# joeyee/Onet

Hardware: AMD Instinct MI355X
Metric: training images/sec (twin 256x256 pass) (higher is better)
Workload: dtype f32

## Files before the change

### include/onet_hip.h

```cpp
#ifndef ONET_HIP_H
#define ONET_HIP_H

#include <stdint.h>

#ifdef __cplusplus
extern "C" {
#endif

#define ONET_OK 0
#define ONET_EINVAL (-1)
#define ONET_EHIP (-2)

const char* onet_last_error(void);
int onet_abi_version(void);
int onet_device_info(int* cu_count, int* lds_bytes, int* wave_size, char* arch, int arch_len);

int onet_conv3x3_pack_weights(const float* w, float* wp_fwd, float* wp_dgrad,
                              int Cout, int Cin, void* stream);
int onet_convT2x2_pack_weights(const float* w, float* wp_fwd, float* wp_dgrad,
                               int Cin, int Cout, void* stream);
int onet_convT2x2_pack_weights_fused(const float* w, float* wq, int Cin, int Cout, void* stream);
int onet_convT2x2_fwd(const float* x, int64_t x_bs, const float* wq, const float* bias, float* y, int64_t y_bs,
                      int B, int Cin, int Ct, int h, int w, int Ho, int Wo, int pt, int pl, int operand_bf16,
        void* stream);
// ... 116 lines not shown
int onet_bn_bwd_finalize(const float* part2, int nparts, int64_t count, float* dgamma, float* dbeta, float* coef, int accumulate,
                         int groups, int C, const float* save, const void* da_amax, void* dz_amax, void* stream);
int onet_bn_bwd_finalize_cm(const float* part2, int nparts, int64_t c_stride, int64_t count, float* dgamma,
                            float* dbeta, float* coef, int accumulate, int C, void* stream);
int onet_bn_relu_bwd_apply(const float* da, int64_t da_bs, const float* z, int64_t z_bs, const float* save, const float* coef,
                           float* dz, int64_t dz_bs, void* amax, int group_images, int B, int C, int HW, void* stream);
int onet_bn_relu_apply_split(const void* z, int z_bf16, int64_t z_bs, void* xs, int64_t xs_bs, float* a, int64_t a_bs, const float* save,
                             const void* act_amax, int nparts, int group_images, int B, int C, int H, int W, void* stream);
int onet_bn_relu_apply_pool_split(const void* z, int z_bf16, int64_t z_bs, void* xs, int64_t xs_bs, float* a, int64_t a_bs, void* ys, int64_t ys_bs,
                                  float* y, int64_t y_bs, const float* save, const void* act_amax, int nparts, int group_images, int B, int C,
                                  int H, int W, void* stream);
int onet_bn_bwd_bound(const float* save, const float* coef, const void* da_amax, int64_t count, void* dz_amax, int C, void* stream);
int onet_bn_relu_bwd_apply_split(const float* da, int64_t da_bs, const void* z, int z_bf16, int64_t z_bs, const float* save, const float* coef,
                                 void* dzs, int64_t dzs_bs, const void* dz_amax, int nparts, int group_images, int B, int C, int H, int W,
                                 void* stream);

int onet_maxpool2_fwd(const float* x, int64_t x_bs, float* y, int64_t y_bs,
                      int B, int C, int H, int W, void* stream);
int onet_maxpool2_bwd(const float* x, int64_t x_bs, const float* dy, int64_t dy_bs, const float* add, int64_t add_bs,
                      const float* add2, int64_t add2_bs, float* dx, int64_t dx_bs, int B, int C, int H, int W, int accumulate,
                      void* stream);
int onet_maxpool2_bwd_bn_bands(int H, int W);
int onet_maxpool2_bwd_add_bnreduce(const float* x, int64_t x_bs, const float* dy, int64_t dy_bs, const float* add, int64_t add_bs,
                                        const float* add2, int64_t add2_bs, float* dx, int64_t dx_bs, const void* z, int z_bf16, int64_t z_bs,
                                        const float* save, int group_images, float* part2, void* dx_amax, int B, int C, int H, int W,
                                        void* stream);

int onet_pixel_shuffle2_bias(const float* sub, const float* bias, float* y, int64_t y_bs,
                             int B, int C, int h, int w, int Ho, int Wo, int pt, int pl, void* stream);
int onet_space_to_depth2(const float* dy, int64_t dy_bs, float* sub, float* dbias, double* scratch,
// ... 5 lines not shown
int onet_bilinear2x_fwd(const float* x, int64_t x_bs, float* y, int64_t y_bs, int B, int C,
                        int h, int w, int Ho, int Wo, int pt, int pl, void* stream);
int onet_bilinear2x_bwd(const float* dy, int64_t dy_bs, float* dx, int64_t dx_bs, int B, int C,
                        int h, int w, int Ho, int Wo, int pt, int pl, void* stream);

int onet_complement_clip(const float* x, float* y, float bias, int64_t n, void* stream);

int onet_head_softmax_fwd(const float* Lt, int64_t Lt_bs, const float* Ht, int64_t Ht_bs, const float* Ld, int64_t Ld_bs, const float* Hd,
                          int64_t Hd_bs, float* Vt, float* Vd, float* S, float* sLt, float* sLd, const float* h_save_t, const float* h_save_d,
                          int B, int C, int HW, void* stream);
int onet_head_softmax_bwd(const float* dVt, const float* dVd, const float* dS, const float* gsLt, const float* gsLd, const float* S,
                          const float* Lt, int64_t Lt_bs, const float* Ht, int64_t Ht_bs, const float* Ld, int64_t Ld_bs, const float* Hd,
                          int64_t Hd_bs, float* dLt, float* dHt, float* dLd, float* dHd, const float* h_save_t, const float* h_save_d, int B,
                          int C, int HW, void* stream);

int onet_jsd_fwd(const float* L, int64_t L_bs, const float* Si, int64_t Si_bs,
                 const float* Sp, int64_t Sp_bs, float* sums, double* part, float* jsd,
                 int B, int C, int HW, void* stream);
int onet_jsd_nparts(void);
int onet_jsd_bwd(const float* gscale, const float* sums, const float* Si, int64_t Si_bs,
                 const float* Sp, int64_t Sp_bs, float* gL, float* dSi, float* dSp,
                 int B, int HW, void* stream);
int onet_log1pexp_inplace(float* x, int64_t n, void* stream);
int onet_log1pexp_bwd(const float* x, const float* g, float* out, int64_t n, void* stream);

int onet_argmax2(const float* S, int64_t* Y, int B, int HW, void* stream);

int onet_normalise_per_frame(const float* x, float* y, int planes, int HW, void* stream);

int onet_clutter_fft_size(void);
// ... 21 lines not shown
```

### onet_amd/csrc/bn.hip

```cpp
#include <type_traits>
#include "common.hpp"

using namespace onet;

__global__ __launch_bounds__(256) void bn_stats_partial_kernel(const float* __restrict__ z, int64_t z_bs,
                                                               float* __restrict__ part, int C, int HW,
                                                               int chunks, int chunk_len) {
    __shared__ double red[16];
    const int c = blockIdx.x % C;
    const int p = blockIdx.x / C;
    const int b = p / chunks, ch = p % chunks;
    const float* src = z + (int64_t)b * z_bs + (int64_t)c * HW;
    const int beg = ch * chunk_len;
    const int end = min(beg + chunk_len, HW);
    const bool vec = ((HW & 3) == 0) && ((z_bs & 3) == 0) && ((chunk_len & 3) == 0);
    const double pivot = (double)src[beg];
    double v[2] = {0.0, 0.0};
    if (vec) {
        int i = beg + threadIdx.x * 4;
        for (; i + 3072 < end; i += 4096) {
            float4 q[4];
#pragma unroll
            for (int k = 0; k < 4; ++k) q[k] = *reinterpret_cast<const float4*>(src + i + 1024 * k);
#pragma unroll
// ... 459 lines not shown
    }
    if (!live) return;
    if (ys) {
        unsigned* o = ys + (int64_t)b * ys_bs;
        bn_store_slots(o, ((int64_t)(c8 * Hp + yo) * np) * Wp + 2 * q, Wp, m[0], s_act, np);
        bn_store_slots(o, ((int64_t)(c8 * Hp + yo) * np) * Wp + 2 * q + 1, Wp, m[1], s_act, np);
    }
    if (yf) {
        float* d = yf + (int64_t)b * yf_bs + (int64_t)c8 * 8 * Hp * Wp + (int64_t)yo * Wp + 2 * q;
#pragma unroll
        for (int k = 0; k < 8; ++k) *reinterpret_cast<float2*>(d + (int64_t)k * Hp * Wp) = make_float2(m[0][k], m[1][k]);
    }
}

constexpr int BN_BWD_OCC16 = 4;
template <typename ZT = float>
__global__ __launch_bounds__(256, sizeof(ZT) == 2 ? BN_BWD_OCC16 : 3) void bn_relu_bwd_apply_split_kernel(const float* __restrict__ da, int64_t da_bs, const ZT* __restrict__ z,
                                                                      int64_t z_bs, const float* __restrict__ save, const float* __restrict__ coef,
                                                                      unsigned* __restrict__ dzs, int64_t dzs_bs, const unsigned* __restrict__ slots,
                                                                      int C, int H, int W, int bpp, int np, int gimg) {
    float inv;
    const float s = np == 1 ? 1.f : amax_scale(amax_read(slots), true, inv);
    const int plane = blockIdx.x / bpp, blk = blockIdx.x % bpp;
    const int C8 = C >> 3, b = plane / C8, c8 = plane % C8;
    if (gimg) {
        save += (int64_t)(b / gimg) * 4 * C;
        if (coef) coef += (int64_t)(b / gimg) * 4 * C;
    }
    bn_u32x4* const tr = bn_tr_lds();
    const int HW = H * W, p = (blk * 256 + threadIdx.x) * 4;
    const bool live = p < HW;
    const ZT* zs = z + (int64_t)b * z_bs + (int64_t)c8 * 8 * HW + p;
    const float* ds = da + (int64_t)b * da_bs + (int64_t)c8 * 8 * HW + p;
    constexpr bool Z16 = sizeof(ZT) == 2;
    typename std::conditional<Z16, uint2, float4>::type zq[8];
    float4 gq[8];
#pragma unroll
    for (int k = 0; k < 8; ++k) {
        if constexpr (Z16) zq[k] = live ? *reinterpret_cast<const uint2*>(zs + (int64_t)k * HW) : make_uint2(0u, 0u);
        else zq[k] = live ? *reinterpret_cast<const float4*>(zs + (int64_t)k * HW) : make_float4(0.f, 0.f, 0.f, 0.f);
        gq[k] = live ? *reinterpret_cast<const float4*>(ds + (int64_t)k * HW) : make_float4(0.f, 0.f, 0.f, 0.f);
    }
    float v[4][8];
#pragma unroll
    for (int k = 0; k < 8; ++k) {
        const int c = c8 * 8 + k;
        const float mean = save[c], invstd = save[C + c], sc = save[2 * C + c], sh = save[3 * C + c];
        const double c1 = coef ? (double)coef[c] + (double)coef[C + c] : 0.0;
        const double c2 = coef ? (double)coef[2 * C + c] + (double)coef[3 * C + c] : 0.0;
        float zz[4];
        if constexpr (Z16) {
            zz[0] = __builtin_bit_cast(float, zq[k].x << 16); zz[1] = __builtin_bit_cast(float, zq[k].x & 0xffff0000u);
            zz[2] = __builtin_bit_cast(float, zq[k].y << 16); zz[3] = __builtin_bit_cast(float, zq[k].y & 0xffff0000u);
        } else {
            zz[0] = zq[k].x; zz[1] = zq[k].y; zz[2] = zq[k].z; zz[3] = zq[k].w;
        }
        const float gg[4] = {gq[k].x, gq[k].y, gq[k].z, gq[k].w};
#pragma unroll
        for (int e = 0; e < 4; ++e) {
            const double dy = fmaf(zz[e] - mean, sc, sh) > 0.f ? (double)gg[e] : 0.0;
            v[e][k] = (float)((double)sc * (dy - c1 - (((double)zz[e] - (double)mean) * (double)invstd) * c2));
        }
    }
    bn_store_slots_block(tr, dzs + (int64_t)b * dzs_bs, c8, H, W, blk * 1024, HW, v, s, np);
}

__global__ __launch_bounds__(64) void bn_bwd_bound_kernel(const float* __restrict__ save, const float* __restrict__ coef,
                                                          const unsigned* __restrict__ da_slots, float xhat_max, unsigned* __restrict__ dz_slots,
                                                          int C) {
    const float da_max = amax_read(da_slots);
    float bound = 0.f;
    for (int c = blockIdx.x * 64 + threadIdx.x; c < C; c += gridDim.x * 64) {
// ... 65 lines not shown
            v[1] += dy * (((double)zi - meand) * invd);
            vmax = fmaxf(vmax, fabsf(ds[i]));
        }
    }
    amax_commit(vmax, amax);
    block_sum_256<double, 2>(v, red);
    if (threadIdx.x == 0) {
        float* o = part2 + ((int64_t)p * C + c) * 4;
        o[0] = (float)v[0];
        o[1] = (float)(v[0] - (double)o[0]);
        o[2] = (float)v[1];
        o[3] = (float)(v[1] - (double)o[2]);
    }
}

__global__ __launch_bounds__(256) void bn_bwd_finalize_kernel(const float* __restrict__ part2, int nparts,
                                                             double count, float* dgamma, float* dbeta,
                                                             float* coef, int accumulate, int C, const float* __restrict__ save = nullptr,
                                                             const unsigned* __restrict__ da_slots = nullptr,
                                                             unsigned* __restrict__ dz_slots = nullptr, float xhat_max = 0.f, int groups = 1) {
    __shared__ double wsum[2][4];
    const float da_max = dz_slots ? amax_read(da_slots) : 0.f;
    const int c = blockIdx.x;
    float acc_b = 0.f, acc_g = 0.f;
    if (accumulate && threadIdx.x == 0) {
        acc_b = dbeta ? dbeta[c] : 0.f;
        acc_g = dgamma ? dgamma[c] : 0.f;
    }
    for (int g = 0; g < groups; ++g) {
        const float* rec = part2 + (int64_t)g * nparts * C * 4;
// ... 283 lines not shown
                 "bn_relu_bwd_apply_split: bad args");
    ONET_REQUIRE((reinterpret_cast<uintptr_t>(dzs) & 15) == 0 && (dzs_bs & 3) == 0 && (reinterpret_cast<uintptr_t>(z) & 15) == 0 && (z_bs & 3) == 0 &&
                 (reinterpret_cast<uintptr_t>(da) & 15) == 0 && (da_bs & 3) == 0, "bn_relu_bwd_apply_split: 16-byte aligned rows and slots required");
    const int bpp = cdiv((int64_t)H * W, 1024);
    const int64_t blocks = (int64_t)B * (C / 8) * bpp;
    ONET_REQUIRE(blocks < (1ll << 31) && (int64_t)H * W < (1 << 24), "bn_relu_bwd_apply_split: grid too large");
    if (z_bf16)
        hipLaunchKernelGGL(bn_relu_bwd_apply_split_kernel<__bf16>, dim3((unsigned)blocks), dim3(256), bn_tr_bytes(nparts), as_stream(stream), da, da_bs,
                           (const __bf16*)z, z_bs, save, coef, (unsigned*)dzs, dzs_bs, (const unsigned*)dz_amax, C, H, W, bpp, nparts, group_images);
    else
        hipLaunchKernelGGL(bn_relu_bwd_apply_split_kernel<float>, dim3((unsigned)blocks), dim3(256), bn_tr_bytes(nparts), as_stream(stream), da, da_bs,
                           (const float*)z, z_bs, save, coef, (unsigned*)dzs, dzs_bs, (const unsigned*)dz_amax, C, H, W, bpp, nparts, group_images);
    return check_launch("bn_relu_bwd_apply_split_kernel");
}

int onet_bn_bwd_finalize_cm(const float* part2, int nparts, int64_t c_stride, int64_t count, float* dgamma, float* dbeta,
                            float* coef, int accumulate, int C, void* stream) {
    ONET_REQUIRE(part2 && nparts > 0 && count > 0 && C > 0 && c_stride >= (int64_t)nparts * 2, "bn_bwd_finalize_cm: bad args");
    hipLaunchKernelGGL(bn_bwd_finalize_cm_kernel, dim3(C), dim3(256), 0, as_stream(stream), part2, nparts, c_stride,
                       (double)count, dgamma, dbeta, coef, accumulate, C);
    return check_launch("bn_bwd_finalize_cm_kernel");
}

int onet_bn_bwd_finalize(const float* part2, int nparts, int64_t count, float* dgamma, float* dbeta, float* coef, int accumulate,
                               int groups, int C, const float* save, const void* da_amax, void* dz_amax, void* stream) {
    ONET_REQUIRE(part2 && nparts > 0 && count > 0 && C > 0 && groups >= 1 && (!dz_amax || (save && da_amax)), "bn_bwd_finalize: bad args");
    hipLaunchKernelGGL(bn_bwd_finalize_kernel, dim3(C), dim3(256), 0, as_stream(stream), part2, nparts, (double)count, dgamma, dbeta, coef,
                       accumulate, C, save, (const unsigned*)da_amax, (unsigned*)dz_amax, sqrtf((float)(count > 1 ? count - 1 : 1)), groups);
    return check_launch("bn_bwd_finalize_kernel");
}
// ... 14 lines not shown
```

### onet_amd/csrc/head_loss.hip

```cpp
#include <algorithm>
#include "common.hpp"

using namespace onet;

__device__ __forceinline__ float f_quirk(float x) {
    if (x <= -37.f) return logf(1.f + expf(expf(x)));
    if (x <= 18.f) return logf(1.f + expf(x));
    if (x < 33.3f) return x + expf(-x);
    return x;
}
__device__ __forceinline__ float df_quirk(float x) {
    if (x <= -37.f) {
        const float e = expf(x), ee = expf(e);
        return ee / (1.f + ee) * e;
    }
    if (x <= 18.f) {
        const float e = expf(x);
        return e / (1.f + e);
    }
    if (x < 33.3f) return 1.f - expf(-x);
    return 1.f;
}

__global__ void log1pexp_kernel(float* x, int64_t n) {
// ... 30 lines not shown
            st_ += a;
            sd_ += d;
        }
        Vt[i] = vt;
        Vd[i] = vd;
        if (sLt) sLt[i] = st_;
        if (sLd) sLd[i] = sd_;
        const float m = fmaxf(vt, vd);
        const float et = expf(vt - m), ed = expf(vd - m);
        const float den = et + ed;
        S[((int64_t)b * 2 + 0) * HW + p] = et / den;
        S[((int64_t)b * 2 + 1) * HW + p] = ed / den;
    }
}

__global__ __launch_bounds__(256) void head_softmax_bwd_kernel(
    const float* __restrict__ dVt, const float* __restrict__ dVd, const float* __restrict__ dS,
    const float* __restrict__ S, const float* __restrict__ Lt, int64_t Lt_bs, const float* __restrict__ Ht,
    int64_t Ht_bs, const float* __restrict__ Ld, int64_t Ld_bs, const float* __restrict__ Hd, int64_t Hd_bs,
    float* __restrict__ dLt, float* __restrict__ dHt, float* __restrict__ dLd, float* __restrict__ dHd,
    const float* __restrict__ gsLt, const float* __restrict__ gsLd, const float* __restrict__ nt, const float* __restrict__ nd, int B,
    int C, int HW) {
    const int64_t n = (int64_t)B * HW;
    const int64_t CHW = (int64_t)C * HW;
    for (int64_t i = blockIdx.x * (int64_t)blockDim.x + threadIdx.x; i < n; i += (int64_t)gridDim.x * blockDim.x) {
        const int b = (int)(i / HW);
        const int p = (int)(i % HW);
        float gt = dVt ? dVt[i] : 0.f, gd = dVd ? dVd[i] : 0.f;
        if (dS) {
            const float st = S[((int64_t)b * 2 + 0) * HW + p], sd = S[((int64_t)b * 2 + 1) * HW + p];
            const float a = dS[((int64_t)b * 2 + 0) * HW + p], d = dS[((int64_t)b * 2 + 1) * HW + p];
            const float t = st * sd * (a - d);
            gt += t;
            gd -= t;
        }
        const float* lt = Lt + b * Lt_bs + p;
        const float* ht = Ht + b * Ht_bs + p;
        const float* ld = Ld + b * Ld_bs + p;
        const float* hd = Hd + b * Hd_bs + p;
        float* olt = dLt + b * CHW + p;
        float* oht = dHt + b * CHW + p;
        float* old_ = dLd + b * CHW + p;
        float* ohd = dHd + b * CHW + p;
        const float at = gsLt ? gsLt[i] : 0.f, ad = gsLd ? gsLd[i] : 0.f;
        for (int c = 0; c < C; ++c) {
            const int64_t o = (int64_t)c * HW;
            float h1 = ht[o], h2 = hd[o];
            if (nt) {
                h1 = fmaxf(fmaf(h1 - nt[c], nt[2 * C + c], nt[3 * C + c]), 0.f);
                h2 = fmaxf(fmaf(h2 - nd[c], nd[2 * C + c], nd[3 * C + c]), 0.f);
            }
            olt[o] = fmaf(gt, h1, at);
            oht[o] = gt * lt[o];
            old_[o] = fmaf(gd, h2, ad);
            ohd[o] = gd * ld[o];
        }
    }
}

constexpr int JSD_BLOCKS = 2048;

__global__ __launch_bounds__(256) void jsd_fwd_kernel(const float* __restrict__ L, int64_t L_bs,
                                                      const float* __restrict__ Si, int64_t Si_bs,
                                                      const float* __restrict__ Sp, int64_t Sp_bs,
                                                      float* __restrict__ sums, double* __restrict__ part, int B,
                                                      int C, int HW) {
    __shared__ double red[4];
    const int64_t n = (int64_t)B * HW;
    double acc[1] = {0.0};
    for (int64_t i = blockIdx.x * (int64_t)blockDim.x + threadIdx.x; i < n; i += (int64_t)gridDim.x * blockDim.x) {
        const int b = (int)(i / HW);
        const int p = (int)(i % HW);
        float sl;
        if (L) {
// ... 73 lines not shown
                       Lt_bs, Ht, Ht_bs, Ld, Ld_bs, Hd, Hd_bs, Vt, Vd, S, sLt, sLd, h_save_t, h_save_d, B, C, HW);
    return check_launch("head_softmax_fwd_kernel");
}

int onet_head_softmax_bwd(const float* dVt, const float* dVd, const float* dS, const float* gsLt, const float* gsLd, const float* S,
                          const float* Lt, int64_t Lt_bs, const float* Ht, int64_t Ht_bs, const float* Ld, int64_t Ld_bs, const float* Hd,
                          int64_t Hd_bs, float* dLt, float* dHt, float* dLd, float* dHd, const float* h_save_t, const float* h_save_d, int B,
                          int C, int HW, void* stream) {
    ONET_REQUIRE(S && Lt && Ht && Ld && Hd && dLt && dHt && dLd && dHd && (!h_save_t == !h_save_d) && B > 0 && C > 0 && HW > 0,
                 "head_softmax_bwd: bad args");
    hipLaunchKernelGGL(head_softmax_bwd_kernel, dim3(grid_px((int64_t)B * HW)), dim3(256), 0, as_stream(stream), dVt,
                       dVd, dS, S, Lt, Lt_bs, Ht, Ht_bs, Ld, Ld_bs, Hd, Hd_bs, dLt, dHt, dLd, dHd, gsLt, gsLd, h_save_t, h_save_d, B, C, HW);
    return check_launch("head_softmax_bwd_kernel");
}

int onet_jsd_nparts(void) { return JSD_BLOCKS; }

int onet_jsd_fwd(const float* L, int64_t L_bs, const float* Si, int64_t Si_bs, const float* Sp, int64_t Sp_bs,
                 float* sums, double* part, float* jsd, int B, int C, int HW, void* stream) {
    ONET_REQUIRE(Si && Sp && sums && part && jsd && B > 0 && C > 0 && HW > 0, "jsd_fwd: bad args");
    const int64_t n = (int64_t)B * HW;
    int blocks = (int)std::min<int64_t>((n + 255) / 256, JSD_BLOCKS);
    hipLaunchKernelGGL(jsd_fwd_kernel, dim3(blocks), dim3(256), 0, as_stream(stream), L, L_bs, Si, Si_bs, Sp, Sp_bs,
                       sums, part, B, C, HW);
    int rc = check_launch("jsd_fwd_kernel");
    if (rc) return rc;
    hipLaunchKernelGGL(jsd_final_kernel, dim3(1), dim3(256), 0, as_stream(stream), (const double*)part, blocks,
                       -1.0 / (double)n, jsd);
    return check_launch("jsd_final_kernel");
}
// ... 29 lines not shown
```

### onet_amd/functional.py

```python
from __future__ import annotations

import torch

from . import ops


def _carries_settings(cls):
    fwd, bwd = cls.forward, cls.backward

    def forward(ctx, *args, **kw):
        ctx._onet_settings = ops.active_settings()
        return fwd(ctx, *args, **kw)

    def backward(ctx, *grads):
        if torch.is_grad_enabled():
            raise RuntimeError("onet_amd: double differentiation (create_graph=True) is not supported: the HIP backward kernels "
                               "build no graph of their own")
        with ops.using(getattr(ctx, "_onet_settings", None)):
            return bwd(ctx, *grads)

    forward.__doc__, backward.__doc__ = fwd.__doc__, bwd.__doc__
    cls.forward, cls.backward = staticmethod(forward), staticmethod(backward)
    return cls

# ... 137 lines not shown
            else:
                pooled = (torch.empty((Bz, C, Hz // 2, Wz // 2), dtype=torch.float32, device=z.device), None, None)
        if training and cm is not None:
            ops.bn_train_coeffs(z[:Bg], gamma, beta, running_mean, running_var, momentum, eps, cm=(cm, 0, cm.shape[1] // G), save=save_all,
                                act_slots=act_slots, groups=G)
        else:
            for g in range(G):
                if training:
                    ops.bn_train_coeffs(z[g * Bg:(g + 1) * Bg], gamma, beta, running_mean, running_var, momentum, eps, save=save_all[g],
                                        act_slots=act_slots)
                else:
                    ops.bn_eval_coeffs(gamma, beta, running_mean, running_var, eps, save=save_all[g])
        gi = Bg if G > 1 else 0
        if defer_head:
            head["z"], head["save"] = z, save_all
            a_amax = None
        elif pooled is not None:
            if not ops.bn_relu_apply_pool_split(z, save_all, aP, a if keep else None, pooled[2], pooled[0], slots=act_slots, group_images=gi):
                raise RuntimeError("onet_amd: pre-split BatchNorm + pooling pass refused a shape ops.pre_layer_ok accepted")
        elif aP is not None:
            ops.bn_relu_apply_split(z, save_all, aP, a=a if keep else None, slots=act_slots, group_images=gi)
        else:
            ops.bn_relu_apply(z, save_all, out=a, amax=a_amax, group_images=gi)
        p16["a"], p16["a_slots"], p16["a_amax"] = aP, act_slots, a_amax
        ctx.x_slots = x_slots
        ctx.up_link = p16.get("up_link")
        ctx.up_want = None if ctx.up_link is None else ctx.up_link.get("want")
        ctx.twin = ops.twin_src_of(x)
        below = (link_in.pop("z"), link_in.pop("save")) if (training and link_in is not None and "z" in link_in) else (None, None)
        ctx.save_for_backward(x, z, save_all, xP, *below)
        ctx.pre = True
        ctx.training = training
        ctx.packed = packed
        ctx.wshape = tuple(weight.shape)
        _record_versions(ctx, weight, gamma, beta)
        ctx.link_out = ctx.link_in = None
        if training and link_out is not None:
            link_out.clear()
            link_out.update(z=z, save=save_all)
            ctx.link_out = link_out
        if below[0] is not None:
            ctx.link_in = link_in
        if pooled is not None and link_out is not None:
            link_out["pooled"] = pooled
        return a

    @staticmethod
    def _retag_twin(ctx, x):
        tw = getattr(ctx, "twin", None)
        if tw is not None and x is not None and ops.twin_src_of(x) is None:
            x._onet_twin_src = [tw[0], tw[1], None]
        return x

    @staticmethod
    def _backward_pre(ctx, da):
        x, z, save_all, xP, z_below, save_below = ctx.saved_tensors
        x = ConvBNReLUFn._retag_twin(ctx, x)
        need_x, need_w, need_g, need_b = ctx.needs_input_grad[:4]
        _check_versions(ctx, (True, True, False))
        pw, pg, pb = ctx.params
        aff = (ops.grad_slot_if_free(pg) if need_g else None, ops.grad_slot_if_free(pb) if need_b else None)
        rec4, da_amax = None, None
        lk = ctx.link_out
        if lk is not None and "rec4" in lk:
            rda, rec4, da_amax = lk.pop("da"), lk.pop("rec4", None), lk.pop("da_amax", None)
            lk.pop("rec", None)
            if rda.data_ptr() != da.data_ptr() or rda.shape != da.shape or rda.stride() != da.stride():
                rec4 = da_amax = None
        nones = (None,) * 12
        if xP is None:
            if need_w and not need_x and x.shape[1] <= 4 and ops.STEM_WGRAD_BN and (not ops.is_placeholder(x) or ops.twin_src_of(x) is not None):
                dw, dgamma, dbeta = ops.stem_wgrad_bn(x, da, z, save_all, ctx.training, ctx.wshape, affine_out=aff, rec4=rec4,
                                                      out=ops.grad_slot_if_free(pw))
                return (None, dw, (dgamma if need_g else None), (dbeta if need_b else None)) + nones
            dz, dgamma, dbeta = ops.bn_relu_bwd_groups(da, z, save_all, ctx.training, affine_out=aff, rec4=rec4)
            dw = ops.conv3x3_wgrad_auto(x, dz, ctx.wshape, out=ops.grad_slot_if_free(pw)) if need_w else None
            dx = ops.conv3x3_auto(dz, ctx.packed, 1) if need_x else None
            return (dx, dw, (dgamma if need_g else None), (dbeta if need_b else None)) + nones
        dzP, dz_slots, dgamma, dbeta = ops.bn_relu_bwd_split(da, z, save_all, ctx.training, need_affine_grads=(need_g or need_b),
                                                             affine_out=aff, rec4=rec4, da_amax=da_amax)
        s1, s2, sc = ops._slots3(getattr(ctx, "x_slots", None))
        dw = ops.conv3x3_split_wgrad_pre(xP, dzP, ctx.wshape, out=ops.grad_slot_if_free(pw), x_slots=s1, dz_slots=dz_slots, x_slots2=s2,
                                         split_ch=sc) if need_w else None
        dpack = ctx.packed.get_pack("split" if dzP.shape[3] == 2 else "plain16")[1]
        dx = None
        if need_x and z_below is not None and save_below is not None and ctx.training:
            fused = ops.conv3x3_split_dgrad_pre_bnreduce(dzP, dpack, ctx.wshape[1], z_below, save_below, slots=dz_slots,
                                                         always=dz_slots is not None, want_amax=ops.p16_parts() == 2)
            if fused is not None:
                dx, rec_below, am_below = fused
                ctx.link_in["da"], ctx.link_in["rec4"] = dx, rec_below
                if am_below is not None:
                    ctx.link_in["da_amax"] = am_below
        up = getattr(ctx, "up_link", None)
        if need_x and dx is None and up is not None and ctx.up_want and (dz_slots is not None or dzP.shape[3] == 1):
# ... 345 lines not shown
            torch.empty(ctx.shape, dtype=ref.dtype, device=ref.device)
        if g0 is not None:
            out[:B].copy_(g0)
        if g1 is not None:
            out[B:].copy_(g1)
        return out


@_carries_settings
class HeadSoftmaxTwinFn(torch.autograd.Function):

    @staticmethod
    def forward(ctx, L, H, head_link=None):
        B = L.shape[0] // 2
        ctx.h_save = None
        if head_link is not None and "z" in head_link:
            z, save = head_link.pop("z"), head_link.pop("save")
            assert z.shape == H.shape and z.dtype == torch.float32 and save.shape[0] == 2
            ctx.h_save = save
            H = z
        elif ops.is_placeholder(H):
            raise RuntimeError("onet_amd: the head received a placeholder for the last activation without its pre-activation")
        nrm = None if ctx.h_save is None else (ctx.h_save[0], ctx.h_save[1])
        Vt, Vd, S, sLt, sLd = ops.head_softmax_fwd(L[:B], H[:B], L[B:], H[B:], want_sums=True, h_norm=nrm)
        ctx.save_for_backward(L, H, S)
        return Vt, Vd, S, sLt, sLd

    @staticmethod
    def backward(ctx, dVt, dVd, dS, gsLt, gsLd):
        L, H, S = ctx.saved_tensors
        B = L.shape[0] // 2
        nrm = None if ctx.h_save is None else (ctx.h_save[0], ctx.h_save[1])
        dL, dH = ops.head_softmax_bwd(dVt, dVd, dS, S, L[:B], H[:B], L[B:], H[B:], twin=True, gsums=(gsLt, gsLd), h_norm=nrm)
        return dL, dH, None


@_carries_settings
class JSDSumsFn(torch.autograd.Function):

    @staticmethod
    def forward(ctx, sLt, sLd, St, Sd):
        top, _ = ops.jsd_fwd(None, St, Sd, sums=sLt)
        dwn, _ = ops.jsd_fwd(None, Sd, St, sums=sLd)
        ctx.save_for_backward(sLt, sLd, St, Sd)
        return top, dwn

# ... 59 lines not shown
```

### onet_amd/ops.py

```python
from __future__ import annotations

import torch

from . import _lib

F32 = torch.float32


import os as _os


def _flags_from_env():
    out = {}
    for item in _os.environ.get("ONET_FLAGS", "").split(","):
        if "=" in item:
            k, v = item.split("=", 1)
            out[k.strip()] = v.strip()
    return out


_FLAGS = _flags_from_env()


def _flag(name, default):
# ... 1065 lines not shown
        nparts = _bn_nparts(Bg, HW)
        rec4 = torch.empty((G * nparts, C, 4), dtype=F32, device=dev)
        _lib.call("onet_bn_relu_bwd_reduce", _p(da), dabs, _p(z), _z16(z), zbs, _p(save_all), _p(rec4), G * nparts, _p(da_amax), Bg if G > 1 else 0,
                  B, C, HW, _stream(), nbytes=(4 + z.element_size()) * z.numel())
    else:
        assert rec4.shape[0] % G == 0 and rec4.shape[1] == C and rec4.shape[2] == 4 and rec4.is_contiguous()
    og, ob = affine_out if affine_out is not None else (None, None)
    dgamma = torch.empty(C, dtype=F32, device=dev) if og is None else og
    dbeta = torch.empty(C, dtype=F32, device=dev) if ob is None else ob
    coef = torch.empty((G, 4, C), dtype=F32, device=dev) if training else None
    _lib.call("onet_bn_bwd_finalize", _p(rec4), rec4.shape[0] // G, Bg * HW, _p(dgamma), _p(dbeta), _p(coef), 0, G, C, _p(save_all),
              _p(da_amax), _p(dz_slots), _stream())
    return coef, dgamma, dbeta


def bn_relu_bwd_split(da, z, save_all, training, need_affine_grads=True, affine_out=None, rec=None, rec4=None, da_amax=None):
    da, dabs = plane(da)
    z, zbs = plane(z)
    B, C, H, W = z.shape
    G = save_all.shape[0]
    dev = z.device
    np_ = p16_parts()
    dzP = p16_empty(B, C, H, W, dev, np_)
    scaled = np_ == 2
    dz_slots = new_amax(dev) if scaled else None
    if scaled and rec4 is not None and da_amax is None:
        da_amax = absmax_slots(da)
    if rec4 is None:
        da_amax = new_amax(dev) if scaled else None
    coef, dgamma, dbeta = _bn_bwd_groups(da, dabs, z, zbs, save_all, training, affine_out, rec4, da_amax, dz_slots)
    _lib.call("onet_bn_relu_bwd_apply_split", _p(da), dabs, _p(z), _z16(z), zbs, _p(save_all), _p(coef), _p(dzP), _pbs(dzP), _p(dz_slots), np_,
              B // G if G > 1 else 0, B, C, H, W, _stream(), nbytes=(4 + z.element_size() + 2 * np_) * z.numel())
    return dzP, dz_slots, dgamma, dbeta


def stem_wgrad_bn(x, da, z, save_all, training, dw_shape, affine_out=None, rec4=None, out=None, twin=None):
    require_gpu(x, da, z)
    if twin is None:
        twin = twin_src_of(x)
    B, Cin, H, W = x.shape
    x, xbs = plane(twin[0] if twin is not None else x)
    da, dabs = plane(da)
    z, zbs = plane(z)
    Cout = z.shape[1]
    G = save_all.shape[0]
# ... 521 lines not shown
    if twin:
        dL = torch.empty((2 * B, C, H, W), dtype=F32, device=dev)
        dH = torch.empty((2 * B, C, H, W), dtype=F32, device=dev)
        outs = [dL[:B], dH[:B], dL[B:], dH[B:]]
    else:
        outs = [torch.empty((B, C, H, W), dtype=F32, device=dev) for _ in range(4)]
    gst = None if gsums[0] is None else gsums[0].contiguous()
    gsd = None if gsums[1] is None else gsums[1].contiguous()
    nt, nd = h_norm if h_norm is not None else (None, None)
    _lib.call("onet_head_softmax_bwd", _p(dVt), _p(dVd), _p(dS), _p(gst), _p(gsd), _p(S), _p(Lt), a, _p(Ht), b,
              _p(Ld), c, _p(Hd), d, _p(outs[0]), _p(outs[1]), _p(outs[2]), _p(outs[3]), _p(nt), _p(nd), B, C, H * W, _stream(),
              nbytes=32 * Lt.numel())
    return (dL, dH) if twin else outs


def _rows(t):
    B, C, H, W = t.shape
    assert C == 1
    ok = (W == 1 or t.stride(3) == 1) and (H == 1 or t.stride(2) == W)
    if not ok:
        t = t.contiguous()
    return t, (t.stride(0) if B > 1 else H * W)


def jsd_fwd(L, Si, Sp, sums=None):
    require_gpu(Si, Sp)
    Si, ibs = _rows(Si)
    Sp, pbs = _rows(Sp)
    if sums is not None:
        B, _, H, W = sums.shape
# ... 61 lines not shown
```

Baseline: 581.1.

## Fuse head softmax backward with last BN-ReLU backward reduction

The head backward now computes a per-pixel gradient map g once, then a single kernel writes dL and at the same time accumulates the BatchNorm backward partial sums for the last conv unit. dH = g*L is never written out; the BN-ReLU apply kernel recomputes it on the fly from g and L. This removes one full-resolution write and read of dH plus a separate BN reduction pass. In exchange it adds a handoff protocol between the head and the conv unit with placeholder checks, and an extra load of L in the apply kernel.

```diff
diff --git a/include/onet_hip.h b/include/onet_hip.h
--- a/include/onet_hip.h
+++ b/include/onet_hip.h
@@ -154,6 +154,9 @@
 int onet_bn_relu_bwd_apply_split(const float* da, int64_t da_bs, const void* z, int z_bf16, int64_t z_bs, const float* save, const float* coef,
                                  void* dzs, int64_t dzs_bs, const void* dz_amax, int nparts, int group_images, int B, int C, int H, int W,
                                  void* stream);
+int onet_bn_relu_bwd_apply_split_gl(const float* L, int64_t L_bs, const float* g, const float* z, int64_t z_bs, const float* save,
+                                    const float* coef, void* dzs, int64_t dzs_bs, const void* dz_amax, int nparts, int group_images, int B, int C,
+                                    int H, int W, void* stream);
 
 int onet_maxpool2_fwd(const float* x, int64_t x_bs, float* y, int64_t y_bs,
                       int B, int C, int H, int W, void* stream);
@@ -189,6 +192,10 @@
                           int64_t Hd_bs, float* dLt, float* dHt, float* dLd, float* dHd, const float* h_save_t, const float* h_save_d, int B,
                           int C, int HW, void* stream);
 
+int onet_head_grad_map(const float* dVt, const float* dVd, const float* dS, const float* S, float* g, int B, int HW, void* stream);
+int onet_head_bwd_reduce(const float* L, int64_t L_bs, const float* z, int64_t z_bs, const float* g, const float* gsLt, const float* gsLd,
+                         const float* save, float* dL, float* part2, int nparts, void* da_amax, int B, int C, int HW, void* stream);
+
 int onet_jsd_fwd(const float* L, int64_t L_bs, const float* Si, int64_t Si_bs,
                  const float* Sp, int64_t Sp_bs, float* sums, double* part, float* jsd,
                  int B, int C, int HW, void* stream);
diff --git a/onet_amd/csrc/bn.hip b/onet_amd/csrc/bn.hip
--- a/onet_amd/csrc/bn.hip
+++ b/onet_amd/csrc/bn.hip
@@ -497,11 +497,12 @@
 }
 
 constexpr int BN_BWD_OCC16 = 4;
-template <typename ZT = float>
+template <typename ZT = float, bool GL = false>
 __global__ __launch_bounds__(256, sizeof(ZT) == 2 ? BN_BWD_OCC16 : 3) void bn_relu_bwd_apply_split_kernel(const float* __restrict__ da, int64_t da_bs, const ZT* __restrict__ z,
                                                                       int64_t z_bs, const float* __restrict__ save, const float* __restrict__ coef,
                                                                       unsigned* __restrict__ dzs, int64_t dzs_bs, const unsigned* __restrict__ slots,
-                                                                      int C, int H, int W, int bpp, int np, int gimg) {
+                                                                      int C, int H, int W, int bpp, int np, int gimg,
+                                                                      const float* __restrict__ gmap = nullptr) {
     float inv;
     const float s = np == 1 ? 1.f : amax_scale(amax_read(slots), true, inv);
     const int plane = blockIdx.x / bpp, blk = blockIdx.x % bpp;
@@ -518,6 +519,10 @@
     constexpr bool Z16 = sizeof(ZT) == 2;
     typename std::conditional<Z16, uint2, float4>::type zq[8];
     float4 gq[8];
+    float4 g4 = make_float4(0.f, 0.f, 0.f, 0.f);
+    if constexpr (GL) {
+        if (live) g4 = *reinterpret_cast<const float4*>(gmap + (int64_t)b * HW + p);
+    }
 #pragma unroll
     for (int k = 0; k < 8; ++k) {
         if constexpr (Z16) zq[k] = live ? *reinterpret_cast<const uint2*>(zs + (int64_t)k * HW) : make_uint2(0u, 0u);
@@ -538,7 +543,10 @@
         } else {
             zz[0] = zq[k].x; zz[1] = zq[k].y; zz[2] = zq[k].z; zz[3] = zq[k].w;
         }
-        const float gg[4] = {gq[k].x, gq[k].y, gq[k].z, gq[k].w};
+        float gg[4] = {gq[k].x, gq[k].y, gq[k].z, gq[k].w};
+        if constexpr (GL) {
+            gg[0] *= g4.x; gg[1] *= g4.y; gg[2] *= g4.z; gg[3] *= g4.w;
+        }
 #pragma unroll
         for (int e = 0; e < 4; ++e) {
             const double dy = fmaf(zz[e] - mean, sc, sh) > 0.f ? (double)gg[e] : 0.0;
@@ -634,6 +642,72 @@
     }
 }
 
+__global__ __launch_bounds__(256) void head_bwd_reduce_kernel(const float* __restrict__ L, int64_t L_bs, const float* __restrict__ z,
+                                                              int64_t z_bs, const float* __restrict__ g, const float* __restrict__ at_t,
+                                                              const float* __restrict__ at_d, const float* __restrict__ save,
+                                                              float* __restrict__ dL, float* __restrict__ part2, int C, int HW, int chunks,
+                                                              int chunk_len, unsigned* __restrict__ amax, int gimg) {
+    __shared__ double red[8];
+    float vmax = 0.f;
+    const int c = blockIdx.x % C;
+    const int p = blockIdx.x / C;
+    const int b = p / chunks, ch = p % chunks;
+    save += (int64_t)(b / gimg) * 4 * C;
+    const float mean = save[c], invstd = save[C + c], sc = save[2 * C + c], sh = save[3 * C + c];
+    const double meand = mean, invd = invstd;
+    const float* zs = z + (int64_t)b * z_bs + (int64_t)c * HW;
+    const float* ls = L + (int64_t)b * L_bs + (int64_t)c * HW;
+    const float* gs = g + (int64_t)b * HW;
+    const float* as = b < gimg ? at_t : at_d;
+    if (as) as += (int64_t)(b % gimg) * HW;
+    float* os = dL + ((int64_t)b * C + c) * HW;
+    const int beg = ch * chunk_len, end = min(beg + chunk_len, HW);
+    const float4 zero4 = make_float4(0.f, 0.f, 0.f, 0.f);
+    double v[2] = {0.0, 0.0};
+    auto four = [&](const float4& q, const float4& l, const float4& gv, const float4& av) -> float4 {
+        const float zz[4] = {q.x, q.y, q.z, q.w}, ll[4] = {l.x, l.y, l.z, l.w}, gg[4] = {gv.x, gv.y, gv.z, gv.w}, aa[4] = {av.x, av.y, av.z, av.w};
+        float o[4];
+#pragma unroll
+        for (int e = 0; e < 4; ++e) {
+            const float x = fmaf(zz[e] - mean, sc, sh);
+            o[e] = fmaf(gg[e], fmaxf(x, 0.f), aa[e]);
+            const float da = gg[e] * ll[e];
+            const double dy = x > 0.f ? (double)da : 0.0;
+            v[0] += dy;
+            v[1] += dy * (((double)zz[e] - meand) * invd);
+            vmax = fmaxf(vmax, fabsf(da));
+        }
+        return make_float4(o[0], o[1], o[2], o[3]);
+    };
+    int i = beg + threadIdx.x * 4;
+    for (; i + 3072 < end; i += 4096) {
+        float4 q[4], l[4], gv[4], av[4];
+#pragma unroll
+        for (int k = 0; k < 4; ++k) {
+            q[k] = *reinterpret_cast<const float4*>(zs + i + 1024 * k);
+            l[k] = *reinterpret_cast<const float4*>(ls + i + 1024 * k);
+            gv[k] = *reinterpret_cast<const float4*>(gs + i + 1024 * k);
+            av[k] = as ? *reinterpret_cast<const float4*>(as + i + 1024 * k) : zero4;
+        }
+#pragma unroll
+        for (int k = 0; k < 4; ++k) *reinterpret_cast<float4*>(os + i + 1024 * k) = four(q[k], l[k], gv[k], av[k]);
+    }
+    for (; i < end; i += 1024) {
+        const float4 q = *reinterpret_cast<const float4*>(zs + i), l = *reinterpret_cast<const float4*>(ls + i);
+        const float4 gv = *reinterpret_cast<const float4*>(gs + i), av = as ? *reinterpret_cast<const float4*>(as + i) : zero4;
+        *reinterpret_cast<float4*>(os + i) = four(q, l, gv, av);
+    }
+    amax_commit(vmax, amax);
+    block_sum_256<double, 2>(v, red);
+    if (threadIdx.x == 0) {
+        float* o = part2 + ((int64_t)p * C + c) * 4;
+        o[0] = (float)v[0];
+        o[1] = (float)(v[0] - (double)o[0]);
+        o[2] = (float)v[1];
+        o[3] = (float)(v[1] - (double)o[2]);
+    }
+}
+
 __global__ __launch_bounds__(256) void bn_bwd_finalize_kernel(const float* __restrict__ part2, int nparts,
                                                              double count, float* dgamma, float* dbeta,
                                                              float* coef, int accumulate, int C, const float* __restrict__ save = nullptr,
@@ -947,6 +1021,37 @@
     return check_launch("bn_relu_bwd_apply_split_kernel");
 }
 
+int onet_head_bwd_reduce(const float* L, int64_t L_bs, const float* z, int64_t z_bs, const float* g, const float* gsLt, const float* gsLd,
+                         const float* save, float* dL, float* part2, int nparts, void* da_amax, int B, int C, int HW, void* stream) {
+    ONET_REQUIRE(L && z && g && save && dL && part2 && B > 0 && (B % 2) == 0 && C > 0 && HW > 0, "head_bwd_reduce: bad args (B = images of the twin batch)");
+    auto al = [](const void* q) { return (reinterpret_cast<uintptr_t>(q) & 15) == 0; };
+    ONET_REQUIRE((HW & 3) == 0 && (L_bs & 3) == 0 && (z_bs & 3) == 0 && al(L) && al(z) && al(g) && al(gsLt) && al(gsLd) && al(dL),
+                 "head_bwd_reduce: HW %% 4 == 0 and 16-byte aligned rows required");
+    int chunks, chunk_len;
+    ONET_REQUIRE(split_plan(nparts, B, HW, chunks, chunk_len), "head_bwd_reduce: nparts=%d must be a multiple of B=%d", nparts, B);
+    ONET_REQUIRE((int64_t)nparts * C < (1ll << 31), "head_bwd_reduce: grid too large");
+    hipLaunchKernelGGL(head_bwd_reduce_kernel, dim3((unsigned)((int64_t)nparts * C)), dim3(256), 0, as_stream(stream), L, L_bs, z, z_bs, g, gsLt,
+                       gsLd, save, dL, part2, C, HW, chunks, chunk_len, (unsigned*)da_amax, B / 2);
+    return check_launch("head_bwd_reduce_kernel");
+}
+
+int onet_bn_relu_bwd_apply_split_gl(const float* L, int64_t L_bs, const float* g, const float* z, int64_t z_bs, const float* save,
+                                    const float* coef, void* dzs, int64_t dzs_bs, const void* dz_amax, int nparts, int group_images, int B, int C,
+                                    int H, int W, void* stream) {
+    ONET_REQUIRE(nparts == 1 || nparts == 2, "bn_relu_bwd_apply_split_gl: nparts must be 2 (fp16 hi | mid) or 1 (plain bf16)");
+    ONET_REQUIRE(L && g && z && save && dzs && (dz_amax || nparts == 1) && B > 0 && C > 0 && (C % 8) == 0 && H > 0 && W > 0 && (W % 4) == 0,
+                 "bn_relu_bwd_apply_split_gl: bad args");
+    ONET_REQUIRE((reinterpret_cast<uintptr_t>(dzs) & 15) == 0 && (dzs_bs & 3) == 0 && (reinterpret_cast<uintptr_t>(z) & 15) == 0 && (z_bs & 3) == 0 &&
+                 (reinterpret_cast<uintptr_t>(L) & 15) == 0 && (L_bs & 3) == 0 && (reinterpret_cast<uintptr_t>(g) & 15) == 0,
+                 "bn_relu_bwd_apply_split_gl: 16-byte aligned rows and slots required");
+    const int bpp = cdiv((int64_t)H * W, 1024);
+    const int64_t blocks = (int64_t)B * (C / 8) * bpp;
+    ONET_REQUIRE(blocks < (1ll << 31) && (int64_t)H * W < (1 << 24), "bn_relu_bwd_apply_split_gl: grid too large");
+    hipLaunchKernelGGL((bn_relu_bwd_apply_split_kernel<float, true>), dim3((unsigned)blocks), dim3(256), bn_tr_bytes(nparts), as_stream(stream), L, L_bs,
+                       z, z_bs, save, coef, (unsigned*)dzs, dzs_bs, (const unsigned*)dz_amax, C, H, W, bpp, nparts, group_images, g);
+    return check_launch("bn_relu_bwd_apply_split_kernel");
+}
+
 int onet_bn_bwd_finalize_cm(const float* part2, int nparts, int64_t c_stride, int64_t count, float* dgamma, float* dbeta,
                             float* coef, int accumulate, int C, void* stream) {
     ONET_REQUIRE(part2 && nparts > 0 && count > 0 && C > 0 && c_stride >= (int64_t)nparts * 2, "bn_bwd_finalize_cm: bad args");
diff --git a/onet_amd/csrc/head_loss.hip b/onet_amd/csrc/head_loss.hip
--- a/onet_amd/csrc/head_loss.hip
+++ b/onet_amd/csrc/head_loss.hip
@@ -68,6 +68,19 @@
     }
 }
 
+__device__ __forceinline__ void head_px_grad(const float* __restrict__ dVt, const float* __restrict__ dVd, const float* __restrict__ dS,
+                                             const float* __restrict__ S, int64_t i, int b, int p, int HW, float& gt, float& gd) {
+    gt = dVt ? dVt[i] : 0.f;
+    gd = dVd ? dVd[i] : 0.f;
+    if (dS) {
+        const float st = S[((int64_t)b * 2 + 0) * HW + p], sd = S[((int64_t)b * 2 + 1) * HW + p];
+        const float a = dS[((int64_t)b * 2 + 0) * HW + p], d = dS[((int64_t)b * 2 + 1) * HW + p];
+        const float t = st * sd * (a - d);
+        gt += t;
+        gd -= t;
+    }
+}
+
 __global__ __launch_bounds__(256) void head_softmax_bwd_kernel(
     const float* __restrict__ dVt, const float* __restrict__ dVd, const float* __restrict__ dS,
     const float* __restrict__ S, const float* __restrict__ Lt, int64_t Lt_bs, const float* __restrict__ Ht,
@@ -80,14 +93,8 @@
     for (int64_t i = blockIdx.x * (int64_t)blockDim.x + threadIdx.x; i < n; i += (int64_t)gridDim.x * blockDim.x) {
         const int b = (int)(i / HW);
         const int p = (int)(i % HW);
-        float gt = dVt ? dVt[i] : 0.f, gd = dVd ? dVd[i] : 0.f;
-        if (dS) {
-            const float st = S[((int64_t)b * 2 + 0) * HW + p], sd = S[((int64_t)b * 2 + 1) * HW + p];
-            const float a = dS[((int64_t)b * 2 + 0) * HW + p], d = dS[((int64_t)b * 2 + 1) * HW + p];
-            const float t = st * sd * (a - d);
-            gt += t;
-            gd -= t;
-        }
+        float gt, gd;
+        head_px_grad(dVt, dVd, dS, S, i, b, p, HW, gt, gd);
         const float* lt = Lt + b * Lt_bs + p;
         const float* ht = Ht + b * Ht_bs + p;
         const float* ld = Ld + b * Ld_bs + p;
@@ -112,6 +119,18 @@
     }
 }
 
+__global__ __launch_bounds__(256) void head_grad_map_kernel(const float* __restrict__ dVt, const float* __restrict__ dVd,
+                                                            const float* __restrict__ dS, const float* __restrict__ S,
+                                                            float* __restrict__ g, int B, int HW) {
+    const int64_t n = (int64_t)B * HW;
+    for (int64_t i = blockIdx.x * (int64_t)blockDim.x + threadIdx.x; i < n; i += (int64_t)gridDim.x * blockDim.x) {
+        float gt, gd;
+        head_px_grad(dVt, dVd, dS, S, i, (int)(i / HW), (int)(i % HW), HW, gt, gd);
+        g[i] = gt;
+        g[n + i] = gd;
+    }
+}
+
 constexpr int JSD_BLOCKS = 2048;
 
 __global__ __launch_bounds__(256) void jsd_fwd_kernel(const float* __restrict__ L, int64_t L_bs,
@@ -215,6 +234,12 @@
     return check_launch("head_softmax_bwd_kernel");
 }
 
+int onet_head_grad_map(const float* dVt, const float* dVd, const float* dS, const float* S, float* g, int B, int HW, void* stream) {
+    ONET_REQUIRE(g && (S || !dS) && B > 0 && HW > 0, "head_grad_map: bad args");
+    hipLaunchKernelGGL(head_grad_map_kernel, dim3(grid_px((int64_t)B * HW)), dim3(256), 0, as_stream(stream), dVt, dVd, dS, S, g, B, HW);
+    return check_launch("head_grad_map_kernel");
+}
+
 int onet_jsd_nparts(void) { return JSD_BLOCKS; }
 
 int onet_jsd_fwd(const float* L, int64_t L_bs, const float* Si, int64_t Si_bs, const float* Sp, int64_t Sp_bs,
diff --git a/onet_amd/functional.py b/onet_amd/functional.py
--- a/onet_amd/functional.py
+++ b/onet_amd/functional.py
@@ -175,6 +175,7 @@
         gi = Bg if G > 1 else 0
         if defer_head:
             head["z"], head["save"] = z, save_all
+            head["bwd_fuse"] = xP is not None
             a_amax = None
         elif pooled is not None:
             if not ops.bn_relu_apply_pool_split(z, save_all, aP, a if keep else None, pooled[2], pooled[0], slots=act_slots, group_images=gi):
@@ -188,6 +189,7 @@
         ctx.up_link = p16.get("up_link")
         ctx.up_want = None if ctx.up_link is None else ctx.up_link.get("want")
         ctx.twin = ops.twin_src_of(x)
+        ctx.head_link = head if defer_head else None
         below = (link_in.pop("z"), link_in.pop("save")) if (training and link_in is not None and "z" in link_in) else (None, None)
         ctx.save_for_backward(x, z, save_all, xP, *below)
         ctx.pre = True
@@ -214,6 +216,16 @@
         return x
 
     @staticmethod
+    def _take_head_handoff(link, da):
+        if link is None or "gl" not in link:
+            return None
+        rda, rec4, da_amax, gl = link.pop("da"), link.pop("rec4"), link.pop("da_amax", None), link.pop("gl")
+        if not ops.is_placeholder(da) or rda.data_ptr() != da.data_ptr() or rda.shape != da.shape or rda.stride() != da.stride():
+            raise RuntimeError("onet_amd: the head kept the gradient of the last activation unwritten, but autograd handed its unit "
+                               "another tensor (a second consumer of that activation?)")
+        return rec4, da_amax, gl
+
+    @staticmethod
     def _backward_pre(ctx, da):
         x, z, save_all, xP, z_below, save_below = ctx.saved_tensors
         x = ConvBNReLUFn._retag_twin(ctx, x)
@@ -228,6 +240,10 @@
             lk.pop("rec", None)
             if rda.data_ptr() != da.data_ptr() or rda.shape != da.shape or rda.stride() != da.stride():
                 rec4 = da_amax = None
+        da_gl = None
+        hand = ConvBNReLUFn._take_head_handoff(getattr(ctx, "head_link", None), da)
+        if hand is not None:
+            rec4, da_amax, da_gl = hand
         nones = (None,) * 12
         if xP is None:
             if need_w and not need_x and x.shape[1] <= 4 and ops.STEM_WGRAD_BN and (not ops.is_placeholder(x) or ops.twin_src_of(x) is not None):
@@ -239,7 +255,7 @@
             dx = ops.conv3x3_auto(dz, ctx.packed, 1) if need_x else None
             return (dx, dw, (dgamma if need_g else None), (dbeta if need_b else None)) + nones
         dzP, dz_slots, dgamma, dbeta = ops.bn_relu_bwd_split(da, z, save_all, ctx.training, need_affine_grads=(need_g or need_b),
-                                                             affine_out=aff, rec4=rec4, da_amax=da_amax)
+                                                             affine_out=aff, rec4=rec4, da_amax=da_amax, da_gl=da_gl)
         s1, s2, sc = ops._slots3(getattr(ctx, "x_slots", None))
         dw = ops.conv3x3_split_wgrad_pre(xP, dzP, ctx.wshape, out=ops.grad_slot_if_free(pw), x_slots=s1, dz_slots=dz_slots, x_slots2=s2,
                                          split_ch=sc) if need_w else None
@@ -615,10 +631,13 @@
     def forward(ctx, L, H, head_link=None):
         B = L.shape[0] // 2
         ctx.h_save = None
+        ctx.unit_link = None
         if head_link is not None and "z" in head_link:
             z, save = head_link.pop("z"), head_link.pop("save")
             assert z.shape == H.shape and z.dtype == torch.float32 and save.shape[0] == 2
             ctx.h_save = save
+            if head_link.pop("bwd_fuse", False) and ops.is_placeholder(H):
+                ctx.unit_link = head_link
             H = z
         elif ops.is_placeholder(H):
             raise RuntimeError("onet_amd: the head received a placeholder for the last activation without its pre-activation")
@@ -631,6 +650,14 @@
     def backward(ctx, dVt, dVd, dS, gsLt, gsLd):
         L, H, S = ctx.saved_tensors
         B = L.shape[0] // 2
+        lk = ctx.unit_link
+        if lk is not None and ops.HEAD_BWD_FUSE and ctx.needs_input_grad[0] and ctx.needs_input_grad[1] and ops.head_bwd_fuse_ok(L, H):
+            g = ops.head_grad_map(dVt, dVd, dS, S)
+            dL, rec4, da_amax = ops.head_bwd_reduce(g, (gsLt, gsLd), L, H, ctx.h_save, want_amax=ops.p16_parts() == 2)
+            dH = ops.fp32_placeholder(H.shape, H.device)
+            lk.clear()
+            lk.update(da=dH, rec4=rec4, da_amax=da_amax, gl=(g, L))
+            return dL, dH, None
         nrm = None if ctx.h_save is None else (ctx.h_save[0], ctx.h_save[1])
         dL, dH = ops.head_softmax_bwd(dVt, dVd, dS, S, L[:B], H[:B], L[B:], H[B:], twin=True, gsums=(gsLt, gsLd), h_norm=nrm)
         return dL, dH, None
diff --git a/onet_amd/ops.py b/onet_amd/ops.py
--- a/onet_amd/ops.py
+++ b/onet_amd/ops.py
@@ -1103,8 +1103,15 @@
     return coef, dgamma, dbeta
 
 
-def bn_relu_bwd_split(da, z, save_all, training, need_affine_grads=True, affine_out=None, rec=None, rec4=None, da_amax=None):
-    da, dabs = plane(da)
+def bn_relu_bwd_split(da, z, save_all, training, need_affine_grads=True, affine_out=None, rec=None, rec4=None, da_amax=None, da_gl=None):
+    if da_gl is not None:
+        if rec4 is None or _z16(z) or (p16_parts() == 2 and da_amax is None):
+            raise RuntimeError("onet_amd: a BatchNorm backward on an unmaterialised g * L needs the records of the fused head backward")
+        gmap = da_gl[0]
+        da, dabs = plane(da_gl[1])
+        assert gmap.is_contiguous() and gmap.shape[0] == z.shape[0] and gmap.numel() == z.shape[0] * z.shape[2] * z.shape[3] and da.shape == z.shape
+    else:
+        da, dabs = plane(da)
     z, zbs = plane(z)
     B, C, H, W = z.shape
     G = save_all.shape[0]
@@ -1118,6 +1125,10 @@
     if rec4 is None:
         da_amax = new_amax(dev) if scaled else None
     coef, dgamma, dbeta = _bn_bwd_groups(da, dabs, z, zbs, save_all, training, affine_out, rec4, da_amax, dz_slots)
+    if da_gl is not None:
+        _lib.call("onet_bn_relu_bwd_apply_split_gl", _p(da), dabs, _p(gmap), _p(z), zbs, _p(save_all), _p(coef), _p(dzP), _pbs(dzP), _p(dz_slots), np_,
+                  B // G if G > 1 else 0, B, C, H, W, _stream(), nbytes=(8 + 2 * np_) * z.numel() + 4 * gmap.numel())
+        return dzP, dz_slots, dgamma, dbeta
     _lib.call("onet_bn_relu_bwd_apply_split", _p(da), dabs, _p(z), _z16(z), zbs, _p(save_all), _p(coef), _p(dzP), _pbs(dzP), _p(dz_slots), np_,
               B // G if G > 1 else 0, B, C, H, W, _stream(), nbytes=(4 + z.element_size() + 2 * np_) * z.numel())
     return dzP, dz_slots, dgamma, dbeta
@@ -1669,6 +1680,51 @@
     return (dL, dH) if twin else outs
 
 
+HEAD_BWD_FUSE = _flag("HEAD_BWD_FUSE", True)
+
+
+def head_bwd_fuse_ok(L, z):
+    if L.shape != z.shape or z.dtype != F32 or L.dtype != F32 or L.shape[0] % 2 or is_placeholder(L) or is_placeholder(z):
+        return False
+    B, C, H, W = L.shape
+    for t in (L, z):
+        ok = (W == 1 or t.stride(3) == 1) and (H == 1 or t.stride(2) == W) and (C == 1 or t.stride(1) == H * W) and t.stride(0) >= C * H * W
+        if not ok or t.stride(0) % 4 or t.data_ptr() % 16:
+            return False
+    return (H * W) % 4 == 0 and W % 4 == 0 and C % 8 == 0
+
+
+def head_grad_map(dVt, dVd, dS, S):
+    B, _, H, W = S.shape
+    dVt = None if dVt is None else dVt.contiguous()
+    dVd = None if dVd is None else dVd.contiguous()
+    dS = None if dS is None else dS.contiguous()
+    S = S.contiguous()
+    g = torch.empty((2 * B, 1, H, W), dtype=F32, device=S.device)
+    _lib.call("onet_head_grad_map", _p(dVt), _p(dVd), _p(dS), _p(S), _p(g), B, H * W, _stream(),
+              nbytes=4.0 * B * H * W * (2 + (dVt is not None) + (dVd is not None) + 4 * (dS is not None)))
+    return g
+
+
+def head_bwd_reduce(g, gsums, L, z, save_all, want_amax=True):
+    require_gpu(g, L, z)
+    L, lbs = plane(L)
+    z, zbs = plane(z)
+    B2, C, H, W = L.shape
+    HW = H * W
+    dev = L.device
+    assert save_all.shape == (2, 4, C) and save_all.is_contiguous() and g.is_contiguous() and g.numel() == B2 * HW
+    gst = None if gsums[0] is None else gsums[0].contiguous()
+    gsd = None if gsums[1] is None else gsums[1].contiguous()
+    dL = torch.empty((B2, C, H, W), dtype=F32, device=dev)
+    nparts = 2 * _bn_nparts(B2 // 2, HW)
+    rec4 = torch.empty((nparts, C, 4), dtype=F32, device=dev)
+    da_amax = new_amax(dev) if want_amax else None
+    _lib.call("onet_head_bwd_reduce", _p(L), lbs, _p(z), zbs, _p(g), _p(gst), _p(gsd), _p(save_all), _p(dL), _p(rec4), nparts, _p(da_amax),
+              B2, C, HW, _stream(), nbytes=12.0 * L.numel() + 4.0 * B2 * HW * (1 + (gst is not None)))
+    return dL, rec4, da_amax
+
+
 def _rows(t):
     B, C, H, W = t.shape
     assert C == 1
```

Result: faster. 588.9 (median of 6 runs) (+1.3%).
